# tesseract-robotics/trajopt

Measured on AMD Instinct MI355X. Metric: SQP iters/s (+ QP solves/s), 7-DOF x 30-wp x 1024-batch glass_upright, higher is better.
Workload: dtype f64; 1 GPU; config 1: glass_upright 7-DOF 30-waypoint, collision cost, batch=1024 random seeds per GPU; n_dof=7, n_steps=30, batch_per_gpu=1024, qp_n=572, qp_m=876, parallelism=seeds sharded, dp1

## Files before the change

### trajopt_amd/csrc/tmx_api.cpp

```cpp
#include <algorithm>
#include <cstddef>
#include <limits>
#include <string>
#include <vector>

#include "tmx_kernels.h"
#include "tmx_wave_kernels.h"
#include "tmx_wave_plan.h"
#include "tmx_row_perm.h"
#include "tmx_upload.h"

#ifdef TMX_HOST_EMU
#include <chrono>
thread_local tmx_emu_idx tmx_emu_threadIdx, tmx_emu_blockIdx, tmx_emu_blockDim, tmx_emu_gridDim;
thread_local double* tmx_emu_smem = nullptr;
double tmx_emu_now_ms()
{
  return std::chrono::duration<double, std::milli>(std::chrono::steady_clock::now().time_since_epoch()).count();
}
#else
#include <rccl/rccl.h>
#endif

#define HIPCHK(call)                                                                                                  \
// ... 1402 lines not shown
      const int c = L.wp_start[t + 1] - L.wp_start[t];
      for (int u = L.wp_start[t]; u < L.wp_start[t + 1]; ++u)
        pl.epos[L.wp_list[u]] = acc + (u - L.wp_start[t]);
      acc += c + (c & 1);
      rows_max = std::max(rows_max, c);
    }
    for (int r = 0; r < R; ++r)
      naux_max = std::max(naux_max, L.naux[r]);
    pl.setup_fast = (rows_max <= TMX_SETUP_COL && naux_max <= 2 && R <= 2 * TMX_QP_NT) ? 1 : 0;
    pl.polish_fast = 0;
    if (pl.setup_fast && dpart_fits(D, T) && R2 == 0)
    {
      DPart dp;
      dpart_make(T, dp);
      const size_t gn = (size_t)dp.Lmax * D, g_doubles = (size_t)dp.P * gn * dpart_gstride((int)gn);
      pl.polish_fast = polish_fast_doubles(T, D * T, R, NA, acc + TMX_SETUP_COL) <= g_doubles ? 1 : 0;
    }
    const size_t eval_room = tmx_eval_scratch_doubles(R, D * T, (int)L.vel_first.size(), L.n_costs, L.n_cnts);
    pl.step_fast = (pl.setup_fast && dpart_fits(D, T) && R >= 1 && 2 * (size_t)L.n_costs + 3 * (size_t)L.n_cnts + TMX_STEP_LOG_HEAD + 1 <= eval_room && R2 == 0 && D * T <= TMX_QP_NT && P.n_max + 1 <= TMX_STEP_CP_PASSES * TMX_QP_NT && P.flavor == 0 &&
                    !P.st && !P.band && !P.band_rows && !E.qp_dense && !P.use_time && P.n_fx == 0 && P.n_stencil == 0 && P.n_tt == 0 && P.n_tv == 0 &&
                    !(pl.coef_far & 2))
                       ? 1
                       : 0;
  }
  pl.smem_small = small_smem_bytes(L, P);
#if TMX_IS_DEVICE
  {
    std::vector<int> plan(TMX_WV_NT * TMX_WV_REC, 0);
    int gmax = 4, aux2 = 0, n3 = 0;
    if (hooks.wave == '1' && P.flavor == 0 && R2 == 0 && pl.coef_far == 0 && !E.qp_dense && !P.st && !P.band && !P.use_time && P.n_fx == 0 &&
        wave_plan_build(D, T, R, L.st.data(), L.naux.data(), plan.data(), &gmax, &aux2, &n3))
    {
      const size_t lds = std::max(pl.smem_small, wave_lds_doubles(D, T, R) * sizeof(double));
      if (lds <= 40 * 1024)
      {
        pl.plan.swap(plan);
        pl.wave_ok = 1;
        pl.wv_gmax = gmax;
        pl.wv_aux2 = aux2;
        pl.smem_wave = lds;
      }
    }
  }
#endif
  pl.smem_qp = qp_smem_bytes(D, T, R, NA, R2, pl.coef_far);
  if (P.tt_chain > 0 || P.tv_chain)
// ... 98 lines not shown
  UP(ls_link, L.ls_link);
  UP(ls_center, L.ls_center);
  UP(ls_radius, L.ls_radius);
  UP(ob_center, L.ob_center);
  UP(ob_radius, L.ob_radius);
  UP(ob_axis, L.ob_axis);
  UP(tv_owner, L.tv_owner);
  UP(tv_joint, L.tv_joint);
  UP(tv_first, L.tv_first);
  UP(tv_last, L.tv_last);
  UP(tv_coeff, L.tv_coeff);
  UP(tv_target, L.tv_target);
  UP(tv_up, L.tv_up);
  UP(tv_lo, L.tv_lo);
  UP(tt_owner, L.tt_owner);
  UP(tt_form, L.tt_form);
  UP(tt_slot, L.tt_slot);
  UP(tt_coeff, L.tt_coeff);
  UP(tt_limit, L.tt_limit);
  P.coef_far = pl.coef_far;
  P.setup_fast = pl.setup_fast;
  P.polish_fast = pl.polish_fast;
  P.step_fast = pl.step_fast;
  P.tt_place = pl.tt_place;
  P.wave_ok = pl.wave_ok;
  P.wv_gmax = pl.wv_gmax;
  P.wv_aux2 = pl.wv_aux2;
  if (!pl.row_perm.empty())
    UP(row_perm, pl.row_perm);
  UP(wp_pst, pl.pst);
  UP(row_epos, pl.epos);
  if (pl.wave_ok)
    UP(wv_plan, pl.plan);
#undef UP
  if (!ctx->dp)
  {
    void* p = nullptr;
    HIPCHK(hipMalloc(&p, sizeof(DevProblem)));
    ctx->dp = static_cast<DevProblem*>(p);
  }
  HIPCHK(hipMemcpy(ctx->dp, &P, sizeof(DevProblem), hipMemcpyHostToDevice));
  return TMX_OK;
}

static tmx_status configure_launch(tmx_ctx* ctx, const DevProblem& P, const Lowered& L, const EngineChoice& E, const Placement& pl, const UploadHooks& hooks)
{
// ... 1472 lines not shown
}

__attribute__((visibility("default"))) int tmx_debug_setup_fast(tmx_ctx* ctx)
{
  if (!ctx || !ctx->have_problem)
    return -1;
  return ctx->hp.setup_fast;
}

__attribute__((visibility("default"))) int tmx_debug_polish_fast(tmx_ctx* ctx)
{
  if (!ctx || !ctx->have_problem)
    return -1;
  return ctx->hp.polish_fast;
}

__attribute__((visibility("default"))) int tmx_debug_step_fast(tmx_ctx* ctx)
{
  if (!ctx || !ctx->have_problem)
    return -1;
  return ctx->hp.step_fast;
}

__attribute__((visibility("default"))) int tmx_debug_wave_ok(tmx_ctx* ctx)
{
  if (!ctx || !ctx->have_problem)
    return -1;
  return ctx->hp.wave_ok;
}

__attribute__((visibility("default"))) int tmx_debug_qp_dense(tmx_ctx* ctx)
{
  if (!ctx || !ctx->have_problem)
    return -1;
  return ctx->hp.qp_dense;
}

__attribute__((visibility("default"))) int tmx_debug_tt_chain(tmx_ctx* ctx)
{
  if (!ctx || !ctx->have_problem)
    return -1;
  return ctx->hp.tt_chain;
}

__attribute__((visibility("default"))) int tmx_debug_tv_chain(tmx_ctx* ctx)
{
// ... 23 lines not shown
```

### trajopt_amd/csrc/tmx_kernels.h

```cpp
#pragma once
#include "tmx_solve.h"
#include "tmx_step.h"
#include "tmx_generic.h"

#define TMX_WORK(smem, Bt) ((Bt)->ws_hbm ? (Bt)->ws_hbm + (size_t)blockIdx.x * (size_t)(Bt)->ws_hbm_stride : (smem))

template <bool HULL>
TMX_DEVFN void prepare_body(const DevProblem* P, const DevBatch* Bt)
{
  TMX_SMEM(smem);
  const int b = blockIdx.x, tid = threadIdx.x, NT = blockDim.x;
  const int NX = P->NX, D = P->D, R = P->R;
  const double* x0 = Bt->x0 + (size_t)b * NX;
  double* x = Bt->x + (size_t)b * NX;
  for (int v = tid; v < NX; v += NT)
  {
    const int j = v % D;
    double y = fmax(P->jl[j] + 1e-6, x0[v]);
    y = fmin(P->ju[j] - 1e-6, x0[v]);
    x[v] = (P->flavor == 1) ? x0[v] : y;
  }
  int* act = Bt->active + (size_t)b * R;
  for (int r = tid; r < R; r += NT)
    act[r] = 0;
// ... 348 lines not shown
TMX_DEVFN void sqp_step_block(const DevProblem* P, const DevBatch* Bt, int b, double* smem, int tid, int NT, double* chain_lds = nullptr)
{
  const int R = P->R, D = P->D, NX = P->NX;
  int* act = Bt->active + (size_t)b * R;
  double* coef = Bt->coef + (size_t)b * R * D;
  double* rhs = Bt->rhs + (size_t)b * R;
  double* x = Bt->x + (size_t)b * NX;
  double* xn = Bt->xnew + (size_t)b * NX;
  const double* xq = Bt->xq + (size_t)b * P->n_max;
#ifdef TMX_PROFILE
  long long tp0 = TMX_CLK();
  const long long wall0 = wall_clock64();
#endif
  if (P->sqp.max_time < 1e300)
  {
    if (tid == 0)
      sqp_time_limit_check(P, Bt, b);
    TMX_SYNC();
    if (Bt->phase[b] == PHASE_DONE)
      return;
  }
  if (Bt->phase[b] == PHASE_CONVEXIFY)
  {
    convexify_terms(P, x, act, coef, Bt->coef2 + (size_t)b * P->n_link * D, rhs, smem, tid, NT, Bt->rowc + (size_t)b * R, Bt->qdyn + (size_t)b * NX);
#ifdef TMX_PROFILE
    if (tid == 0)
    {
      const long long tnow = TMX_CLK();
      Bt->prof[(size_t)b * 16 + 4] += tnow - tp0;
      tp0 = tnow;
    }
#endif
#if TMX_IS_DEVICE
    if (TMX_UNI_B(!HBM && NT == TMX_QP_NT && P->step_fast != 0 && !(P->dbg_flags & 8) && TMX_FAST_ALLOWED))
    {
#if TMX_ADMM_OUTLINED && !(defined(TMX_PROFILE) && defined(TMX_FINE))
      unsigned lds_off = (unsigned)(size_t)smem;
      TMX_ASM_OPAQUE_SGPR(lds_off);
      qp_structure_fast_nl(P, Bt, b, lds_off);
#else
      qp_structure_fast(P, act, coef, Bt->dims + 4 * b, Bt->hashes + 4 * b, reinterpret_cast<int*>(smem), tid TMX_F5_ARGS(&tp0, Bt->prof + (size_t)b * 16));
#endif
    }
    else
#endif
    {
      QpWs cwd;
      qp_structure(P, act, coef, Bt->coef2 + (size_t)b * P->n_link * D, rhs, x, Bt->trust[b], Bt->merit + (size_t)b * P->n_cnts, Bt->dims + 4 * b,
                   Bt->hashes + 4 * b, nullptr, reinterpret_cast<int*>(smem), tid, NT, Bt->qdyn + (size_t)b * NX, compact_lists_of(cwd, P, Bt, b),
                   nullptr, nullptr, nullptr, nullptr TMX_F5_ARGS(&tp0, Bt->prof + (size_t)b * 16));
    }
#if TMX_LINK_ROWS
    if (P->flavor == 1)
      sqp2_begin_qp(P, Bt, b, smem, tid, NT);
#endif
  }
  TMX_SYNC();
#ifdef TMX_PROFILE
  if (tid == 0)
    Bt->prof[(size_t)b * 16 + 11] += TMX_CLK() - tp0;
#endif
  qp_solve_block<HBM, BANDK, false>(P, Bt, b, smem, tid, NT, chain_lds);
#ifdef TMX_PROFILE
  tp0 = TMX_CLK();
#endif
  for (int v = tid; v < NX; v += NT)
    xn[v] = xq[v];
  TMX_SYNC();
  evaluate_terms(P, xn, Bt->new_cost_vals + (size_t)b * P->n_costs, Bt->new_cnt_viols + (size_t)b * P->n_cnts, smem, tid, NT);
#if defined(TMX_PROFILE) && defined(TMX_FINE) && TMX_FINE == 5
  [[maybe_unused]] long long* const f5_tl = &tp0;
  [[maybe_unused]] long long* const f5_pc = Bt->prof + (size_t)b * 16;
#endif
  TMX_F5_TICK(13);
#if TMX_IS_DEVICE
  if (TMX_UNI_B(!HBM && NT == TMX_QP_NT && P->step_fast != 0 && !(P->dbg_flags & 8) && TMX_FAST_ALLOWED))
  {
#if TMX_ADMM_OUTLINED && !(defined(TMX_PROFILE) && defined(TMX_FINE))
    unsigned lds_off = (unsigned)(size_t)smem;
    TMX_ASM_OPAQUE_SGPR(lds_off);
    sqp_update_fast_nl(P, Bt, b, lds_off);
#else
    sqp_update_fast(P, Bt, b, smem, tid TMX_F5_ARGS(&tp0, Bt->prof + (size_t)b * 16));
#endif
  }
  else
#endif
#if TMX_LINK_ROWS
  if (P->flavor == 1)
    sqp2_update_block(P, Bt, b, smem, tid, NT);
  else
#endif
    sqp_update_block(P, Bt, b, smem, tid, NT TMX_F5_ARGS(&tp0, Bt->prof + (size_t)b * 16));
  TMX_SYNC();
#ifdef TMX_PROFILE
  if (tid == 0)
  {
    Bt->prof[(size_t)b * 16 + 12] += TMX_CLK() - tp0;
    Bt->prof[(size_t)b * 16 + 1] += wall_clock64() - wall0;
  }
#endif
}

TMX_KERNEL_LB2(TMX_QP_NT, TMX_QP_WGS_PER_CU) k_sqp_fused(const DevProblem* P, const DevBatch* Bt, int max_steps)
{
  TMX_SMEM(smem);
// ... 307 lines not shown
```

### trajopt_amd/csrc/tmx_step.h

```cpp
#pragma once
#include "tmx_solve.h"

#define TMX_STEP_CP_PASSES 6

#if TMX_IS_DEVICE
TMX_DEVFN void qp_structure_fast(const DevProblem* P, const int* active, const double* coef, int* dims, unsigned long long* hashes,
                                 int* iscratch, int tid TMX_F5_PARAMS)
{
  constexpr int NT = TMX_QP_NT;
  const int D = P->D, NX = P->NX, R = P->R;
  int* colptr = iscratch;
  int* rowref = colptr + P->n_max + 1;
  int* auxref = rowref + R;
  int* lact = auxref + R;
  int* lnaux = lact + R;
  int* ccount = lnaux + R;
  int acc_off = 2 * (P->n_max + 1) + 4 * R;
  acc_off += (acc_off & 1);
  unsigned long long* acc = reinterpret_cast<unsigned long long*>(iscratch + acc_off);
  int* scan = iscratch + acc_off + 16;
  int* nm = scan + TMX_STEP_CP_PASSES * (NT / 64);
  for (int r = tid; r < R; r += NT)
  {
    lact[r] = active[r] ? 1 : 0;
// ... 134 lines not shown
  };
  if (pv)
  {
    int pos = cp[0];
#pragma unroll
    for (int k = 0; k < TMX_SETUP_COL; ++k)
      if (mask & (1u << k))
      {
        row_term(rref[k], pos);
        ++pos;
      }
    row_term(mg + v, pos);
  }
  for (int r = tid; r < R; r += NT)
    if (lact[r])
      for (int k = 0; k < lnaux[r]; ++k)
      {
        const int col = auxref[r] + k;
        const int pos = colptr[col];
        row_term(rowref[r], pos);
        row_term(mg + col, pos + 1);
      }
  TMX_F5_TICK(6);
  unsigned long long hP = 0ULL, wsP = 0ULL;
  {
    const int pp_bytes = n + 1, pp_full = pp_bytes / 8, pp_rem = pp_bytes % 8;
    const int pi_full = P->nnzP / 8, pi_rem = P->nnzP % 8;
    auto p_term = [&](long long row, int run) {
      hP += tmx_hash_term(row, (uint64_t)run, 2);
      if (run < pi_full)
        wsP += tmx_hash_term(row, (uint64_t)run, 12);
      else if (run == pi_full && pi_rem > 0)
        wsP += tmx_hash_term((long long)((unsigned long long)row & ((1ULL << (8 * pi_rem)) - 1ULL)), (uint64_t)run, 12);
    };
    for (int c = tid; c <= n; c += NT)
    {
      int run = (c <= NX) ? P->p_colptr[c] : P->nnzP;
      const long long val = run;
      hP += tmx_hash_term(val, (uint64_t)c, 1);
      if (c < pp_full)
        wsP += tmx_hash_term(val, (uint64_t)c, 11);
      else if (c == pp_full && pp_rem > 0)
        wsP += tmx_hash_term((long long)((unsigned long long)val & ((1ULL << (8 * pp_rem)) - 1ULL)), (uint64_t)c, 11);
      if (c < NX)
      {
        if (c >= D && P->po[c - D] != 0.0)
        {
          p_term(c - D, run);
          ++run;
        }
        if (P->pd[c] != 0.0)
          p_term(c, run);
      }
    }
  }
  TMX_ATOMIC_ADD_U64(&acc[0], hP);
  TMX_ATOMIC_ADD_U64(&acc[1], hA);
  TMX_ATOMIC_ADD_U64(&acc[2], wsP);
  TMX_ATOMIC_ADD_U64(&acc[3], wsA);
  TMX_SYNC();
  if (tid == 0)
  {
    hashes[0] = acc[0];
    hashes[1] = acc[1];
    hashes[2] = acc[2];
    hashes[3] = acc[3];
  }
  TMX_SYNC();
}

TMX_DEVFN void sqp_update_fast(const DevProblem* P, const DevBatch* Bt, int b, double* smem, int tid TMX_F5_PARAMS)
{
  constexpr int NT = TMX_QP_NT;
  const int NX = P->NX, nc = P->n_costs, nv = P->n_cnts;
  double* model_cost = smem;
  double* model_viol = smem + nc;
  double* l_cost = model_viol + nv;
  double* l_new_cost = l_cost + nc;
  double* l_viol = l_new_cost + nc;
  double* l_new_viol = l_viol + nv;
  double* l_merit = l_new_viol + nv;
  double* head = l_merit + nv;
  double* cost_vals = Bt->cost_vals + (size_t)b * nc;
  double* cnt_viols = Bt->cnt_viols + (size_t)b * nv;
  const double* new_cost = Bt->new_cost_vals + (size_t)b * nc;
  const double* new_viol = Bt->new_cnt_viols + (size_t)b * nv;
  const double* merit = Bt->merit + (size_t)b * nv;
  const bool solved = Bt->cvx[b] == TMX_CVX_SOLVED && Bt->phase[b] != PHASE_DONE;
  if (solved)
    sqp_model_values<false>(P, Bt, b, Bt->xq + (size_t)b * P->n_max, smem, tid, NT);
  TMX_F5_TICK(14);
  for (int k = tid; k < nc; k += NT)
  {
    l_cost[k] = cost_vals[k];
    l_new_cost[k] = new_cost[k];
  }
  for (int k = tid; k < nv; k += NT)
  {
    l_viol[k] = cnt_viols[k];
    l_new_viol[k] = new_viol[k];
    l_merit[k] = merit[k];
  }
  if (tid == 0)
    head[TMX_STEP_LOG_HEAD] = 0.0;
  TMX_SYNC();
  if (tid == 0)
  {
    Bt->accept_flag[b] = 0;
    const DecideIo io = { l_cost, l_viol, l_new_cost, l_new_viol, l_merit, head };
    sqp_decide_io(P, Bt, b, model_cost, model_viol, io);
  }
  TMX_SYNC();
// ... 33 lines not shown
    for (int k = tid; k < nv; k += NT)
      cnt_viols[k] = l_new_viol[k];
  }
}

#if TMX_ADMM_OUTLINED
__device__ __attribute__((noinline)) static void qp_structure_fast_nl(const DevProblem* P_in, const DevBatch* Bt_in, int b_in, unsigned lds_in)
{
  const DevProblem* P = tmx_uniform_ptr(P_in);
  const DevBatch* Bt = tmx_uniform_ptr(Bt_in);
  const int b = __builtin_amdgcn_readfirstlane(b_in);
  const int tid = threadIdx.x;
  double* smem = (double*)(tmx_lds_d*)(size_t)(unsigned)__builtin_amdgcn_readfirstlane((int)lds_in);
  qp_structure_fast(P, Bt->active + (size_t)b * P->R, Bt->coef + (size_t)b * P->R * P->D, Bt->dims + 4 * b, Bt->hashes + 4 * b,
                    reinterpret_cast<int*>(smem), tid);
}
__device__ __attribute__((noinline)) static void sqp_update_fast_nl(const DevProblem* P_in, const DevBatch* Bt_in, int b_in, unsigned lds_in)
{
  const DevProblem* P = tmx_uniform_ptr(P_in);
  const DevBatch* Bt = tmx_uniform_ptr(Bt_in);
  const int b = __builtin_amdgcn_readfirstlane(b_in);
  const int tid = threadIdx.x;
  double* smem = (double*)(tmx_lds_d*)(size_t)(unsigned)__builtin_amdgcn_readfirstlane((int)lds_in);
  sqp_update_fast(P, Bt, b, smem, tid);
}
#endif
#endif
```

### trajopt_amd/csrc/tmx_terms.h

```cpp
#pragma once
#include "tmx_types.h"
#include "../../include/tmx_detmath.h"
#include "../../include/tmx_expr.h"
#include "../../include/tmx_geom.h"

#define TMX_EPS_FD 1e-5
#define TMX_CLEANUP_TOL 1e-7

struct Tf3
{
  double R[9];
  double t[3];
};

TMX_DEVFN void tf_from12(const double* a, Tf3& T)
{
  for (int r = 0; r < 3; ++r)
  {
    for (int c = 0; c < 3; ++c)
      T.R[3 * r + c] = a[4 * r + c];
    T.t[r] = a[4 * r + 3];
  }
}
TMX_DEVFN void tf_mul(const Tf3& A, const Tf3& B, Tf3& C)
{
  for (int r = 0; r < 3; ++r)
  {
    for (int c = 0; c < 3; ++c)
      C.R[3 * r + c] = A.R[3 * r + 0] * B.R[0 + c] + A.R[3 * r + 1] * B.R[3 + c] + A.R[3 * r + 2] * B.R[6 + c];
    C.t[r] = A.R[3 * r + 0] * B.t[0] + A.R[3 * r + 1] * B.t[1] + A.R[3 * r + 2] * B.t[2] + A.t[r];
  }
}
TMX_DEVFN void tf_inv(const Tf3& A, Tf3& C)
{
  for (int r = 0; r < 3; ++r)
    for (int c = 0; c < 3; ++c)
      C.R[3 * r + c] = A.R[3 * c + r];
  for (int r = 0; r < 3; ++r)
    C.t[r] = -(C.R[3 * r + 0] * A.t[0] + C.R[3 * r + 1] * A.t[1] + C.R[3 * r + 2] * A.t[2]);
}
TMX_DEVFN void tf_joint_motion(const double* ax, int type, double q, Tf3& T)
{
  for (int k = 0; k < 9; ++k)
    T.R[k] = 0.0;
  T.R[0] = T.R[4] = T.R[8] = 1.0;
  T.t[0] = T.t[1] = T.t[2] = 0.0;
  if (type == 0)
  {
    double c, s;
    tmx_sincos(q, &s, &c);
    const double v = 1.0 - c;
    const double x = ax[0], y = ax[1], z = ax[2];
    T.R[0] = c + x * x * v;
    T.R[1] = x * y * v - z * s;
    T.R[2] = x * z * v + y * s;
    T.R[3] = y * x * v + z * s;
    T.R[4] = c + y * y * v;
    T.R[5] = y * z * v - x * s;
    T.R[6] = z * x * v - y * s;
    T.R[7] = z * y * v + x * s;
    T.R[8] = c + z * z * v;
  }
  else
  {
    T.t[0] = ax[0] * q;
    T.t[1] = ax[1] * q;
    T.t[2] = ax[2] * q;
  }
}

template <class QAt, class Visit>
TMX_DEVFN void fk_link_visit(const DevProblem* P, QAt&& qat, int upto, Tf3& out, Visit&& visit)
{
  Tf3 T, O, M, U;
  tf_from12(P->base, T);
  for (int k = 0; k <= upto; ++k)
  {
    tf_from12(P->origin[k], O);
    tf_mul(T, O, U);
    visit(k, U);
    tf_joint_motion(P->axis[k], P->jtype[k], qat(k), M);
    tf_mul(U, M, T);
  }
  out = T;
}
template <class QAt>
TMX_DEVFN void fk_link_at(const DevProblem* P, QAt&& qat, int upto, Tf3& out)
{
  fk_link_visit(P, qat, upto, out, [](int, const Tf3&) {});
}
TMX_DEVFN void fk_link(const DevProblem* P, const double* q, int upto, Tf3& out)
// ... 161 lines not shown
__device__ __attribute__((noinline)) static int link_closest_b_nl(const double* c, const double* e, const double* oc, const double* oa, const double* ob,
                                                                  const double* mesh, double* p, double* q)
{
  return tmx_link_closest_to_obstacle_b(c, e, oc, oa, ob, mesh, p, q);
}
__device__ __attribute__((noinline)) static double swept_closest_b_nl(const double* ca, const double* e, const double* oc, const double* oa,
                                                                      const double* ob, const double* mesh, double* q, int* inside)
{
  return tmx_swept_closest_to_obstacle_b(ca, e, oc, oa, ob, mesh, q, inside);
}
__device__ __attribute__((noinline)) static int hull_closest_nl(const double* hv, int nv, const double* R0, const double* t0, const double* R1,
                                                                const double* t1, const double* oc, const double* oa, const double* ob,
                                                                const double* mesh, double* p, double* q, double* tau)
{
  return tmx_hull_closest_to_obstacle(hv, nv, R0, t0, R1, t1, oc, oa, ob, mesh, p, q, tau);
}
#else
#define link_closest_b_nl tmx_link_closest_to_obstacle_b
#define swept_closest_b_nl tmx_swept_closest_to_obstacle_b
#define hull_closest_nl tmx_hull_closest_to_obstacle
#endif

template <bool HULL = false>
TMX_DEVFN double contact_distance(const DevProblem* P, const double* q, int s, int o, double n[3], double pw[3])
{
  Tf3 L;
  const int link = P->ls_link[s];
  fk_link(P, q, link, L);
  if constexpr (HULL)
    if (P->n_ls_hull > 0 && P->ls_hull[2 * s + 1] > 0)
    {
      double pc[3], oq[3];
      const int inside = hull_closest_nl(P->hull + 3 * P->ls_hull[2 * s], P->ls_hull[2 * s + 1], L.R, L.t, nullptr, nullptr, P->ob_center + 3 * o,
                                         P->ob_axis + 3 * o, P->n_ob_box > 0 ? P->ob_box + 12 * o : nullptr, P->mesh, pc, oq, nullptr);
      const double len = tmx_contact_normal(pc, oq, inside, n);
      const double rs = P->ls_radius[s];
      for (int r = 0; r < 3; ++r)
        pw[r] = pc[r] + rs * n[r];
      return len - rs - P->ob_radius[o];
    }
  double c[3], d[3];
  for (int r = 0; r < 3; ++r)
    c[r] = L.R[3 * r + 0] * P->ls_center[3 * s + 0] + L.R[3 * r + 1] * P->ls_center[3 * s + 1] +
           L.R[3 * r + 2] * P->ls_center[3 * s + 2] + L.t[r];
  double oq[3];
  int inside = 0;
  if (P->n_ls_capsule > 0 || P->n_ob_box > 0)
  {
    double e[3], pc[3];
    bool capsule = false;
    if (P->n_ls_capsule > 0)
    {
      for (int r = 0; r < 3; ++r)
        e[r] = L.R[3 * r + 0] * P->ls_axis[3 * s + 0] + L.R[3 * r + 1] * P->ls_axis[3 * s + 1] + L.R[3 * r + 2] * P->ls_axis[3 * s + 2];
      capsule = P->ls_axis[3 * s + 0] != 0.0 || P->ls_axis[3 * s + 1] != 0.0 || P->ls_axis[3 * s + 2] != 0.0;
    }
    inside = link_closest_b_nl(c, capsule ? e : nullptr, P->ob_center + 3 * o, P->ob_axis + 3 * o,
                                            P->n_ob_box > 0 ? P->ob_box + 12 * o : nullptr, P->mesh, pc, oq);
    for (int r = 0; r < 3; ++r)
      c[r] = pc[r];
  }
  else
    tmx_obstacle_closest_to_point(P->ob_center + 3 * o, P->ob_axis + 3 * o, c, oq);
  (void)d;
  const double len = tmx_contact_normal(c, oq, inside, n);
  const double rs = P->ls_radius[s];
  for (int r = 0; r < 3; ++r)
    pw[r] = c[r] + rs * n[r];
  return len - rs - P->ob_radius[o];
}

struct LvsContact
{
  double distance, n[3], p_local[3], cc_time;
  double R0[9], R1[9];
};
TMX_DEVFN double lin_spaced_at(int size, double low, double high, int i)
{
  const int size1 = size - 1;
  const double step = (high - low) / (double)size1;
  const bool flip = fabs(high) < fabs(low);
  if (flip)
    return (i == 0) ? low : (high - (double)(size1 - i) * step);
  return (i == size1) ? high : (low + (double)i * step);
}
template <bool HULL = false>
TMX_DEVFN bool lvs_contact(const DevProblem* P, const double* q0, const double* q1, int r, LvsContact& c)
{
  const int s = P->slot_sub[r], o = P->slot_sub2[r], flags = P->slot_sub3[r];
  const int i = (flags >> 3) & 0x1FFF, kmax = flags >> 16;
  const bool fixed0 = flags & 1, fixed1 = flags & 2, cast = flags & 4;
  const double lvs = P->slot_aux3[r], margin = P->slot_aux1[r], buffer = P->slot_aux2[r];
// ... 1449 lines not shown
```

### trajopt_amd/csrc/tmx_types.h

```cpp
#pragma once
#include "../../include/tmx.h"
#include "tmx_platform.h"

enum
{
  SLOT_FIXED = 0,
  SLOT_CARTPOSE = 1,
  SLOT_JOINTPOS = 2,
  SLOT_COLLISION = 3,
  SLOT_JOINTPOS_INEQ = 4,
  SLOT_JOINTVEL = 5,
  SLOT_JOINTVEL_INEQ = 6,
  SLOT_COLLISION_LVS = 7,
  SLOT_FUNC = 9,
  SLOT_CARTVEL = 8,
  SLOT_JOINTVEL_TIME = 10,
  SLOT_TOTAL_TIME = 11
};
#ifndef TMX_LINK_ROWS
#define TMX_LINK_ROWS 1
#endif

enum
{
// ... 57 lines not shown
  int* ls_hull;
  double* hull;
  int n_ls_hull;
  int DK;
  int use_time;
  int n_tv;
  int *tv_owner, *tv_joint, *tv_first, *tv_last;
  double *tv_coeff, *tv_target, *tv_up, *tv_lo;
  int n_tt;
  int *tt_owner, *tt_form, *tt_slot;
  double *tt_coeff, *tt_limit;
  int wave_ok;
  int wv_gmax;
  int wv_aux2;
  int* wv_plan;
  int* row_perm;
  int dbg_flags;
  int tt_chain, tt_place;
  int tv_chain;
  int *wp_pst, *row_epos;
  int setup_fast;
  int polish_fast;
  int step_fast;
};
TMX_HOSTDEVFN int slot_is_diff(int kind) { return kind == SLOT_JOINTVEL || kind == SLOT_JOINTVEL_INEQ; }
#define TMX_TV_REC 5
TMX_HOSTDEVFN int fx_is_quad(int kind) { return kind == 0 || kind == 1 || kind == 3; }
TMX_HOSTDEVFN int fx_is_rows(int kind) { return kind == 2 || kind == 4; }

struct DevBatch
{
  int B, max_rec;
  double *x0, *x, *xnew;
  double *cost_vals, *cnt_viols, *new_cost_vals, *new_cnt_viols, *merit;
  double *trust, *total_cost, *prev_rho;
  int *phase, *iter, *merit_inc, *qp_fail, *status, *retval, *n_fe, *n_qp, *cvx, *prev_ok;
  int *active;
  double *coef, *rhs;
  double *qdyn;
  double *rowc;
  int *solver_init;
  double *coef2;
  int *dims;
  unsigned long long *hashes;
  int *prev_dims;
  unsigned long long *prev_ws;
// ... 42 lines not shown
```

### trajopt_amd/csrc/tmx_upload.h

```cpp
#pragma once
#include <cstddef>
#include <cstdlib>
#include <string>
#include <vector>

struct Lowered
{
  std::vector<int> kind, st, sub, sub2, owner, naux, iscnt, iseq;
  std::vector<double> objc, scale, aux1, aux2;
  std::vector<int> c2, sub3;
  std::vector<double> aux3;
  std::vector<int> aoff;
  std::vector<double> pd, po, pq, po2, po3;
  std::vector<int> p_colptr;
  std::vector<int> fx_t, fx_kind, fx_owner, fx_op0, fx_nops, fx_c0, fx_nout, fx_slot0, fx_ci, fx_ops;
  std::vector<double> fx_consts;
  std::vector<int> vel_first, vel_last, vel_cost, vel_kind, cp_t, cp_owner, cp_iscnt, cp_nrows, cp_idx, cp_slot0;
  std::vector<double> vel_coeffs, vel_targets, cp_coeff, cp_target;
  std::vector<int> tv_owner, tv_joint, tv_first, tv_last, tt_owner, tt_form, tt_slot;
  std::vector<double> tv_coeff, tv_target, tv_up, tv_lo, tt_coeff, tt_limit;
  std::vector<int> ls_link, ls_hull;
  std::vector<double> ls_center, ls_radius, ob_center, ob_radius, ob_axis, ls_axis, ob_box, hullv, mesh;
  std::vector<int> wp_start, wp_list;
  int R = 0, R2 = 0, NA = 0;
// ... 28 lines not shown
  static UploadHooks read()
  {
    auto first = [](const char* name) {
      const char* e = std::getenv(name);
      return e ? e[0] : '\0';
    };
    UploadHooks h;
    h.total_time_chain = first("TMX_TOTAL_TIME_CHAIN");
    h.vel_time_chain = first("TMX_VEL_TIME_CHAIN");
    h.force_coef_far = first("TMX_FORCE_COEF_FAR");
    h.force_compact = first("TMX_FORCE_COMPACT");
    h.row_perm = first("TMX_ROW_PERM");
    h.wave = first("TMX_WAVE");
    h.tt_place = first("TMX_TT_PLACE");
    const char* e = std::getenv("TMX_DENSE_QP_MAX_N");
    h.dense_qp_max_n = e ? std::max(1, std::atoi(e)) : 448;
    h.verbose = std::getenv("TMX_VERBOSE") != nullptr;
    return h;
  }
};

struct Placement
{
  int coef_far = 0, setup_fast = 0, polish_fast = 0, step_fast = 0, tt_place = 0;
  int wave_ok = 0, wv_gmax = 2, wv_aux2 = 0;
  std::vector<int> row_perm, pst, epos, plan;
  size_t smem_qp = 0, smem_small = 0, smem_wave = 0;
  size_t tt_scratch = 0;
};
```

Baseline: 170,200 SQP iters/s.

## Fuse term evaluation with model values in fast step path and tabulate P hash

Adds a merged fast path that evaluates cost and constraint terms together with the QP model values in one pass. It computes forward-kinematics frames once per waypoint in LDS with shared sin/cos and reuses them for collision and Cartesian terms. The P-matrix structure hash, which depends only on n, is now precomputed on the host per possible size and looked up instead of being recomputed each iteration. A convexify_fast routine that reuses cached frames for collision gradients is also added. Together these are meant to remove redundant FK and hashing work per SQP step, at the cost of extra LDS use and eligibility checks, with the old path kept as a fallback.

```diff
diff --git a/trajopt_amd/csrc/tmx_api.cpp b/trajopt_amd/csrc/tmx_api.cpp
--- a/trajopt_amd/csrc/tmx_api.cpp
+++ b/trajopt_amd/csrc/tmx_api.cpp
@@ -1448,6 +1448,22 @@
                     !(pl.coef_far & 2))
                        ? 1
                        : 0;
+    bool kinds_ok = true;
+    for (int k : L.kind)
+      kinds_ok = kinds_ok && tmx_step_eval_kind(k);
+    for (int k : L.vel_kind)
+      kinds_ok = kinds_ok && (k == 0 || k == 1);
+    const size_t qp_lds = qp_smem_bytes(D, T, R, NA, R2, pl.coef_far);
+    pl.eval_fast = (pl.step_fast && kinds_ok && qp_lds <= 160 * 1024 &&
+                    tmx_step_eval_doubles(R, D * T, (int)L.vel_first.size(), L.n_costs, L.n_cnts) * sizeof(double) <= qp_lds &&
+                    tmx_cvx_fast_doubles((int)L.cp_t.size(), D, D * T) * sizeof(double) <= qp_lds)
+                       ? 1
+                       : 0;
+    if (pl.eval_fast)
+    {
+      pl.p_hash.assign(2 * (size_t)(P.n_max - P.NX + 1), 0ULL);
+      tmx_build_p_hash_table(L.p_colptr.data(), L.pd.data(), L.po.data(), D, P.NX, P.n_max, P.nnzP, pl.p_hash.data());
+    }
   }
   pl.smem_small = small_smem_bytes(L, P);
 #if TMX_IS_DEVICE
@@ -1592,6 +1608,9 @@
   P.setup_fast = pl.setup_fast;
   P.polish_fast = pl.polish_fast;
   P.step_fast = pl.step_fast;
+  P.eval_fast = pl.eval_fast;
+  if (pl.eval_fast)
+    UP(p_hash, pl.p_hash);
   P.tt_place = pl.tt_place;
   P.wave_ok = pl.wave_ok;
   P.wv_gmax = pl.wv_gmax;
@@ -3110,6 +3129,13 @@
   return ctx->hp.step_fast;
 }
 
+__attribute__((visibility("default"))) int tmx_debug_eval_fast(tmx_ctx* ctx)
+{
+  if (!ctx || !ctx->have_problem)
+    return -1;
+  return ctx->hp.eval_fast;
+}
+
 __attribute__((visibility("default"))) int tmx_debug_wave_ok(tmx_ctx* ctx)
 {
   if (!ctx || !ctx->have_problem)
diff --git a/trajopt_amd/csrc/tmx_eval.h b/trajopt_amd/csrc/tmx_eval.h
--- /dev/null
+++ b/trajopt_amd/csrc/tmx_eval.h
@@ -0,0 +1,485 @@
+#pragma once
+#include "tmx_solve.h"
+
+TMX_HOSTDEVFN void p_hash_column(const int* p_colptr, const double* pd, const double* po, int D, int NX, int nnzP, int n, int c,
+                                 unsigned long long& hP, unsigned long long& wsP)
+{
+  const int pp_bytes = n + 1, pp_full = pp_bytes / 8, pp_rem = pp_bytes % 8;
+  const int pi_full = nnzP / 8, pi_rem = nnzP % 8;
+  auto p_term = [&](long long row, int run) {
+    hP += tmx_hash_term(row, (uint64_t)run, 2);
+    if (run < pi_full)
+      wsP += tmx_hash_term(row, (uint64_t)run, 12);
+    else if (run == pi_full && pi_rem > 0)
+      wsP += tmx_hash_term((long long)((unsigned long long)row & ((1ULL << (8 * pi_rem)) - 1ULL)), (uint64_t)run, 12);
+  };
+  int run = (c <= NX) ? p_colptr[c] : nnzP;
+  const long long val = run;
+  hP += tmx_hash_term(val, (uint64_t)c, 1);
+  if (c < pp_full)
+    wsP += tmx_hash_term(val, (uint64_t)c, 11);
+  else if (c == pp_full && pp_rem > 0)
+    wsP += tmx_hash_term((long long)((unsigned long long)val & ((1ULL << (8 * pp_rem)) - 1ULL)), (uint64_t)c, 11);
+  if (c < NX)
+  {
+    if (c >= D && po[c - D] != 0.0)
+    {
+      p_term(c - D, run);
+      ++run;
+    }
+    if (pd[c] != 0.0)
+      p_term(c, run);
+  }
+}
+
+static inline void tmx_build_p_hash_table(const int* p_colptr, const double* pd, const double* po, int D, int NX, int n_max, int nnzP,
+                                          unsigned long long* tab)
+{
+  for (int n = NX; n <= n_max; ++n)
+  {
+    unsigned long long hP = 0ULL, wsP = 0ULL;
+    for (int c = 0; c <= n; ++c)
+      p_hash_column(p_colptr, pd, po, D, NX, nnzP, n, c, hP, wsP);
+    tab[2 * (n - NX)] = hP;
+    tab[2 * (n - NX) + 1] = wsP;
+  }
+}
+
+TMX_HOSTDEVFN size_t tmx_step_eval_doubles(int R, int NX, int n_vel, int n_costs, int n_cnts)
+{
+  return (size_t)n_costs + (size_t)n_cnts + 2 * ((size_t)R + (size_t)(R + 1) / 2) + (size_t)n_vel * NX + (size_t)n_vel + 14 * (size_t)NX;
+}
+TMX_HOSTDEVFN bool tmx_step_eval_kind(int kind)
+{
+  return kind == SLOT_FIXED || kind == SLOT_CARTPOSE || kind == SLOT_JOINTPOS || kind == SLOT_JOINTPOS_INEQ || kind == SLOT_COLLISION;
+}
+
+#if TMX_IS_DEVICE
+#define TMX_EVAL_LDS_PTR(p) ((tmx_lds_d*)(size_t)(unsigned)__builtin_amdgcn_readfirstlane((int)(unsigned)(size_t)(p)))
+TMX_DEVFN void step_eval_fast(const DevProblem* P, const DevBatch* Bt, int b, double* smem, int tid)
+{
+  constexpr int NT = TMX_QP_NT;
+  const int D = P->D, NX = P->NX, R = P->R, T = P->T, nc = P->n_costs, nv = P->n_cnts, nvel = P->n_vel;
+  const double* xv = Bt->xnew + (size_t)b * NX;
+  const double* xq = Bt->xq + (size_t)b * P->n_max;
+  double* cost_out = Bt->new_cost_vals + (size_t)b * nc;
+  double* viol_out = Bt->new_cnt_viols + (size_t)b * nv;
+  const bool solved = TMX_UNI_B(Bt->cvx[b] == TMX_CVX_SOLVED && Bt->phase[b] != PHASE_DONE);
+  double* model_cost = smem;
+  double* model_viol = smem + nc;
+  double* xval = model_viol + nv;
+  int* xkeys = reinterpret_cast<int*>(xval + R);
+  double* mval = xval + R + (R + 1) / 2;
+  int* mkeys = reinterpret_cast<int*>(mval + R);
+  double* vterm = mval + R + (R + 1) / 2;
+  double* vsum = vterm + (size_t)nvel * NX;
+  tmx_lds_d* const SN = TMX_EVAL_LDS_PTR(vsum + nvel);
+  tmx_lds_d* const CS = SN + NX;
+  tmx_lds_d* const FR = CS + NX;
+  for (int v = tid; v < NX; v += NT)
+    if (P->jtype[v % D] == 0)
+    {
+      double s, c;
+      tmx_sincos(xv[v], &s, &c);
+      SN[v] = s;
+      CS[v] = c;
+    }
+  {
+    const int* act = Bt->active + (size_t)b * R;
+    const double* coef = Bt->coef + (size_t)b * R * D;
+    const double* rhs = Bt->rhs + (size_t)b * R;
+    QpWs wl;
+    qp_ws_carve(wl, smem, smem, Bt->qp_scratch + (size_t)b * Bt->qp_scratch_stride, D, T, R, P->NA, P->n_link, P->coef_far);
+    const int* aux_ref = wl.aux_ref;
+    for (int r = tid; r < R; r += NT)
+    {
+      const int kind = P->slot_kind[r];
+      const int t = P->slot_t[r];
+      if (kind == SLOT_JOINTPOS_INEQ)
+      {
+        const double pos = xv[t * D + P->slot_sub[r]] - P->slot_aux1[r];
+        const double e = (P->slot_sub2[r] == 0) ? (pos - P->slot_aux2[r]) * P->slot_scale[r] : ((pos * -1) + P->slot_aux2[r]) * P->slot_scale[r];
+        xval[r] = (e > 0) ? e : 0.0;
+      }
+      else if (kind == SLOT_JOINTPOS)
+      {
+        const double d = xv[t * D + P->slot_sub[r]] - P->slot_aux1[r];
+        xval[r] = fabs((d * d) * P->slot_scale[r]);
+      }
+      else if (kind == SLOT_FIXED)
+        xval[r] = 0.0;
+      xkeys[r] = (kind == SLOT_FIXED) ? -1 : (P->slot_iscnt[r] ? nc + P->slot_owner[r] : P->slot_owner[r]);
+      if (solved)
+      {
+        double vr = 0.0;
+        int key = -1;
+        if (kind != SLOT_FIXED && act[r])
+        {
+          if (P->slot_iscnt[r])
+          {
+            double aff = 0.0;
+            for (int j = 0; j < D; ++j)
+              aff += coef[r * D + j] * xq[t * D + j];
+            aff -= rhs[r];
+            vr = P->slot_eq[r] ? fabs(aff) : ((aff > 0) ? aff : 0.0);
+            key = nc + P->slot_owner[r];
+          }
+          else
+          {
+            double sacc = 0.0;
+            for (int k = 0; k < P->slot_naux[r]; ++k)
+              sacc += P->slot_objc[r] * xq[aux_ref[r] + k];
+            vr = sacc;
+            key = P->slot_owner[r];
+          }
+        }
+        mval[r] = vr;
+        mkeys[r] = key;
+      }
+    }
+  }
+  for (int v = 0; v < nvel; ++v)
+  {
+    const int pk = P->vel_kind[v];
+    const int first = P->vel_first[v], len = P->vel_last[v] - first + vel_len_adj<false>(pk);
+    for (int e = tid; e < D * len; e += NT)
+    {
+      const int j = e / len, i = first + e % len;
+      const double dv = pk ? xv[i * D + j] : (xv[(i + 1) * D + j] - xv[i * D + j]);
+      const double d = dv - P->vel_targets[v * TMX_MAX_DOF + j];
+      vterm[(size_t)v * NX + e] = (d * d) * P->vel_coeffs[v * TMX_MAX_DOF + j];
+    }
+  }
+  TMX_SYNC();
+  for (int t = tid; t < T; t += NT)
+  {
+    Tf3 F, O, M, U;
+    tf_from12(P->base, F);
+    for (int k = 0; k < D; ++k)
+    {
+      tf_from12(P->origin[k], O);
+      tf_mul(F, O, U);
+      const int type = P->jtype[k];
+      double s = 0.0, c = 1.0;
+      if (type == 0)
+      {
+        s = SN[t * D + k];
+        c = CS[t * D + k];
+      }
+      tf_joint_motion_sc(P->axis[k], type, xv[t * D + k], s, c, M);
+      tf_mul(U, M, F);
+      tmx_lds_d* const o = FR + (size_t)(t * D + k) * 12;
+#pragma unroll
+      for (int i = 0; i < 9; ++i)
+        o[i] = F.R[i];
+#pragma unroll
+      for (int i = 0; i < 3; ++i)
+        o[9 + i] = F.t[i];
+    }
+  }
+  for (int v = (tid + NT - 64) % NT; v < nvel; v += NT)
+  {
+    const int cnt = D * (P->vel_last[v] - P->vel_first[v] + vel_len_adj<false>(P->vel_kind[v]));
+    double sacc = 0;
+    for (int e = 0; e < cnt; ++e)
+      sacc += vterm[(size_t)v * NX + e];
+    vsum[v] = sacc;
+  }
+  TMX_SYNC();
+  auto frame_at = [&](int t, int k, Tf3& L) {
+    tmx_lds_d* const o = FR + (size_t)(t * D + k) * 12;
+#pragma unroll
+    for (int i = 0; i < 9; ++i)
+      L.R[i] = o[i];
+#pragma unroll
+    for (int i = 0; i < 3; ++i)
+      L.t[i] = o[9 + i];
+  };
+  for (int r = tid; r < R; r += NT)
+    if (P->slot_kind[r] == SLOT_COLLISION)
+    {
+      const int s = P->slot_sub[r];
+      Tf3 L;
+      frame_at(P->slot_t[r], P->ls_link[s], L);
+      double n[3], pw[3];
+      const double dist = contact_distance_at<false>(P, L, s, P->slot_sub2[r], n, pw);
+      const double margin = P->slot_aux1[r];
+      double v = 0.0;
+      if (!(dist > margin + P->slot_aux2[r]))
+      {
+        const double pv = margin - dist;
+        v = ((pv > 0) ? pv : 0.0) * P->slot_objc[r];
+      }
+      xval[r] = v;
+    }
+  for (int c = tid; c < P->n_cp; c += NT)
+  {
+    Tf3 tgt, tinv, L, Tl, src;
+    tf_from12(P->cp_target + 12 * c, tgt);
+    tf_inv(tgt, tinv);
+    frame_at(P->cp_t[c], D - 1, L);
+    tf_from12(P->tool, Tl);
+    tf_mul(L, Tl, src);
+    double err[6], ax[3], ang;
+    transform_error(tinv, src, err, ax, ang);
+    const int s0 = P->cp_slot0[c];
+    for (int i = 0; i < P->cp_nrows[c]; ++i)
+    {
+      const int ix = P->cp_idx[6 * c + i];
+      const double e = (ix == 0) ? err[0] : (ix == 1) ? err[1] : (ix == 2) ? err[2] : (ix == 3) ? err[3] : (ix == 4) ? err[4] : err[5];
+      const double cc = P->cp_coeff[6 * c + i];
+      xval[s0 + i] = P->cp_iscnt[c] ? fabs(e * cc) : fabs(e) * cc;
+    }
+  }
+  TMX_SYNC();
+  for (int k = tid; k < nc + nv; k += NT)
+  {
+    double acc = 0.0;
+    for (int r = P->own_lo[k]; r <= P->own_hi[k]; ++r)
+      if (xkeys[r] == k)
+        acc += xval[r];
+    if (k < nc)
+    {
+      for (int v = 0; v < nvel; ++v)
+        if (P->vel_cost[v] == k)
+          acc += vsum[v];
+      cost_out[k] = acc;
+    }
+    else
+      viol_out[k - nc] = acc;
+  }
+  if (solved)
+    for (int k = (tid + NT - 64) % NT; k < nc + nv; k += NT)
+    {
+      double acc = 0.0;
+      for (int r = P->own_lo[k]; r <= P->own_hi[k]; ++r)
+        if (mkeys[r] == k)
+          acc += mval[r];
+      if (k < nc)
+      {
+        for (int v = 0; v < nvel; ++v)
+          if (P->vel_cost[v] == k)
+            acc += vsum[v];
+        model_cost[k] = acc;
+      }
+      else
+        model_viol[k - nc] = acc;
+    }
+  TMX_SYNC();
+}
+#endif
+
+TMX_HOSTDEVFN size_t tmx_cvx_fast_doubles(int n_cp, int D, int NX) { return tmx_cvx_scratch_doubles(n_cp, D) + 28 * (size_t)NX; }
+
+#if TMX_IS_DEVICE
+TMX_DEVFN void convexify_fast(const DevProblem* P, const double* xv, int* active, double* coef, double* rhs, double* scratch, int tid)
+{
+  constexpr int NT = TMX_QP_NT;
+  const int D = P->D, NX = P->NX, T = P->T, n_cp = P->n_cp;
+  double* rec = scratch;
+  double* errv = rec + (size_t)n_cp * (D + 1) * 7;
+  double* Jm = errv + (size_t)n_cp * 6;
+  tmx_lds_d* const SN = TMX_EVAL_LDS_PTR(scratch + tmx_cvx_scratch_doubles(n_cp, D));
+  tmx_lds_d* const CS = SN + NX;
+  tmx_lds_d* const SNP = CS + NX;
+  tmx_lds_d* const CSP = SNP + NX;
+  tmx_lds_d* const FU = CSP + NX;
+  tmx_lds_d* const FL = FU + (size_t)NX * 12;
+  auto frame_put = [&](tmx_lds_d* o, const Tf3& F) {
+#pragma unroll
+    for (int i = 0; i < 9; ++i)
+      o[i] = F.R[i];
+#pragma unroll
+    for (int i = 0; i < 3; ++i)
+      o[9 + i] = F.t[i];
+  };
+  auto frame_get = [&](tmx_lds_d* o, Tf3& F) {
+#pragma unroll
+    for (int i = 0; i < 9; ++i)
+      F.R[i] = o[i];
+#pragma unroll
+    for (int i = 0; i < 3; ++i)
+      F.t[i] = o[9 + i];
+  };
+  for (int v = tid; v < NX; v += NT)
+    if (P->jtype[v % D] == 0)
+    {
+      double s, c;
+      tmx_sincos(xv[v], &s, &c);
+      SN[v] = s;
+      CS[v] = c;
+      if (n_cp > 0)
+      {
+        tmx_sincos(xv[v] + TMX_EPS_FD, &s, &c);
+        SNP[v] = s;
+        CSP[v] = c;
+      }
+    }
+  TMX_SYNC();
+  for (int t = tid; t < T; t += NT)
+  {
+    Tf3 F, O, M, U;
+    tf_from12(P->base, F);
+    for (int k = 0; k < D; ++k)
+    {
+      tf_from12(P->origin[k], O);
+      tf_mul(F, O, U);
+      frame_put(FU + (size_t)(t * D + k) * 12, U);
+      const int type = P->jtype[k];
+      double s = 0.0, c = 1.0;
+      if (type == 0)
+      {
+        s = SN[t * D + k];
+        c = CS[t * D + k];
+      }
+      tf_joint_motion_sc(P->axis[k], type, xv[t * D + k], s, c, M);
+      tf_mul(U, M, F);
+      frame_put(FL + (size_t)(t * D + k) * 12, F);
+    }
+  }
+  for (int item = (tid + NT - 64) % NT; item < n_cp * (D + 1); item += NT)
+  {
+    const int c = item / (D + 1), k = item % (D + 1);
+    const int t = P->cp_t[c];
+    const double* q = xv + t * D;
+    Tf3 tgt, tinv, src, pp;
+    tf_from12(P->cp_target + 12 * c, tgt);
+    tf_inv(tgt, tinv);
+    {
+      Tf3 F, O, M, U, Tl;
+      tf_from12(P->base, F);
+      for (int j = 0; j < D; ++j)
+      {
+        tf_from12(P->origin[j], O);
+        tf_mul(F, O, U);
+        const int type = P->jtype[j];
+        double s = 0.0, cs = 1.0;
+        if (type == 0)
+        {
+          s = (j == k) ? SNP[t * D + j] : SN[t * D + j];
+          cs = (j == k) ? CSP[t * D + j] : CS[t * D + j];
+        }
+        tf_joint_motion_sc(P->axis[j], type, (j == k) ? q[j] + TMX_EPS_FD : q[j], s, cs, M);
+        tf_mul(U, M, F);
+      }
+      tf_from12(P->tool, Tl);
+      tf_mul(F, Tl, src);
+    }
+    tf_mul(tinv, src, pp);
+    double ax[3], ang;
+    if (k < D)
+      rot_err_decomposed(pp.R, ax, ang);
+    else
+    {
+      double err[6];
+      transform_error(tinv, src, err, ax, ang);
+      for (int r = 0; r < 6; ++r)
+        errv[c * 6 + r] = err[r];
+    }
+    double* o = rec + (size_t)item * 7;
+    for (int r = 0; r < 3; ++r)
+    {
+      o[r] = pp.t[r];
+      o[3 + r] = ax[r];
+    }
+    o[6] = ang;
+  }
+  TMX_SYNC();
+  for (int item = tid; item < n_cp * D; item += NT)
+  {
+    const int c = item / D, k = item % D;
+    const double* o0 = rec + ((size_t)c * (D + 1) + D) * 7;
+    const double* o1 = rec + ((size_t)c * (D + 1) + k) * 7;
+    const double a0 = o0[6], a1 = o1[6];
+    double a1c = a1;
+    if (a1 > M_PI_2 && a0 < -M_PI_2)
+      a1c = a1 - 2.0 * M_PI;
+    else if (a1 < -M_PI_2 && a0 > M_PI_2)
+      a1c = a1 + 2.0 * M_PI;
+    for (int i = 0; i < P->cp_nrows[c]; ++i)
+    {
+      const int r = P->cp_idx[6 * c + i];
+      const double diff = (r < 3) ? o1[r] - o0[r] : o1[r] * a1c - o0[r] * a0;
+      Jm[((size_t)c * 6 + i) * D + k] = diff / TMX_EPS_FD;
+    }
+  }
+  for (int r = tid; r < P->R; r += NT)
+  {
+    if (P->slot_kind[r] != SLOT_COLLISION)
+      continue;
+    const int t = P->slot_t[r];
+    const double* q = xv + t * D;
+    const int s = P->slot_sub[r], o = P->slot_sub2[r];
+    const int link = P->ls_link[s];
+    double n[3], pw[3];
+    Tf3 L;
+    frame_get(FL + (size_t)(t * D + link) * 12, L);
+    const double dist = contact_distance_at<false>(P, L, s, o, n, pw);
+    const double margin = P->slot_aux1[r];
+    if (dist > margin + P->slot_aux2[r])
+    {
+      active[r] = 0;
+      for (int k = 0; k < D; ++k)
+        coef[r * D + k] = 0.0;
+      rhs[r] = 0.0;
+      continue;
+    }
+    double* grad = coef + (size_t)r * D;
+    double gq = 0.0;
+    for (int k = 0; k <= link; ++k)
+    {
+      Tf3 F;
+      frame_get(FU + (size_t)(t * D + k) * 12, F);
+      const double g = contact_grad_col(P, k, F, pw, n);
+      grad[k] = g;
+      gq += g * q[k];
+    }
+    for (int k = link + 1; k < D; ++k)
+    {
+      const double g = -1.0 * (n[0] * 0.0 + n[1] * 0.0 + n[2] * 0.0);
+      grad[k] = g;
+      gq += g * q[k];
+    }
+    const double c_dist = (0.0 + (-gq)) + dist;
+    const double viol_const = margin - c_dist;
+    if (P->slot_iscnt[r])
+    {
+      const double cc = P->slot_scale[r];
+      for (int k = 0; k < D; ++k)
+        coef[r * D + k] = (-grad[k]) * cc;
+      rhs[r] = -(viol_const * cc);
+    }
+    else
+    {
+      for (int k = 0; k < D; ++k)
+        coef[r * D + k] = -grad[k];
+      rhs[r] = -viol_const;
+    }
+    active[r] = 1;
+  }
+  TMX_SYNC();
+  for (int item = tid; item < n_cp * 6; item += NT)
+  {
+    const int c = item / 6, i = item % 6;
+    if (i >= P->cp_nrows[c])
+      continue;
+    const double* q = xv + P->cp_t[c] * D;
+    const double* Jr = Jm + ((size_t)c * 6 + i) * D;
+    const double y = errv[c * 6 + P->cp_idx[6 * c + i]];
+    double dot = 0.0;
+    for (int k = 0; k < D; ++k)
+      dot += Jr[k] * q[k];
+    const double cc = P->cp_coeff[6 * c + i];
+    const int r = P->cp_slot0[c] + i;
+    const double constant = (y - dot) * cc;
+    for (int k = 0; k < D; ++k)
+    {
+      const double jv = Jr[k];
+      coef[r * D + k] = (fabs(jv) > TMX_CLEANUP_TOL) ? jv * cc : 0.0;
+    }
+    rhs[r] = -constant;
+    active[r] = 1;
+  }
+  TMX_SYNC();
+}
+#endif
diff --git a/trajopt_amd/csrc/tmx_kernels.h b/trajopt_amd/csrc/tmx_kernels.h
--- a/trajopt_amd/csrc/tmx_kernels.h
+++ b/trajopt_amd/csrc/tmx_kernels.h
@@ -394,7 +394,20 @@
   }
   if (Bt->phase[b] == PHASE_CONVEXIFY)
   {
-    convexify_terms(P, x, act, coef, Bt->coef2 + (size_t)b * P->n_link * D, rhs, smem, tid, NT, Bt->rowc + (size_t)b * R, Bt->qdyn + (size_t)b * NX);
+#if TMX_IS_DEVICE
+    if (TMX_UNI_B(!HBM && NT == TMX_QP_NT && P->step_fast != 0 && P->eval_fast != 0 && !(P->dbg_flags & (8 | 16)) && TMX_FAST_ALLOWED))
+    {
+#if TMX_ADMM_OUTLINED && !(defined(TMX_PROFILE) && defined(TMX_FINE))
+      unsigned lds_off = (unsigned)(size_t)smem;
+      TMX_ASM_OPAQUE_SGPR(lds_off);
+      convexify_fast_nl(P, Bt, b, lds_off);
+#else
+      convexify_fast(P, x, act, coef, rhs, smem, tid);
+#endif
+    }
+    else
+#endif
+      convexify_terms(P, x, act, coef, Bt->coef2 + (size_t)b * P->n_link * D, rhs, smem, tid, NT, Bt->rowc + (size_t)b * R, Bt->qdyn + (size_t)b * NX);
 #ifdef TMX_PROFILE
     if (tid == 0)
     {
@@ -439,21 +452,33 @@
   for (int v = tid; v < NX; v += NT)
     xn[v] = xq[v];
   TMX_SYNC();
-  evaluate_terms(P, xn, Bt->new_cost_vals + (size_t)b * P->n_costs, Bt->new_cnt_viols + (size_t)b * P->n_cnts, smem, tid, NT);
 #if defined(TMX_PROFILE) && defined(TMX_FINE) && TMX_FINE == 5
   [[maybe_unused]] long long* const f5_tl = &tp0;
   [[maybe_unused]] long long* const f5_pc = Bt->prof + (size_t)b * 16;
 #endif
-  TMX_F5_TICK(13);
-#if TMX_IS_DEVICE
-  if (TMX_UNI_B(!HBM && NT == TMX_QP_NT && P->step_fast != 0 && !(P->dbg_flags & 8) && TMX_FAST_ALLOWED))
+#if TMX_IS_DEVICE
+  const bool step_fast = TMX_UNI_B(!HBM && NT == TMX_QP_NT && P->step_fast != 0 && !(P->dbg_flags & 8) && TMX_FAST_ALLOWED);
+  const bool merged = step_fast && TMX_UNI_B(P->eval_fast != 0 && !(P->dbg_flags & 16));
+  if (!merged)
+#endif
+  {
+    evaluate_terms(P, xn, Bt->new_cost_vals + (size_t)b * P->n_costs, Bt->new_cnt_viols + (size_t)b * P->n_cnts, smem, tid, NT);
+    TMX_F5_TICK(13);
+  }
+#if TMX_IS_DEVICE
+  if (step_fast)
   {
 #if TMX_ADMM_OUTLINED && !(defined(TMX_PROFILE) && defined(TMX_FINE))
     unsigned lds_off = (unsigned)(size_t)smem;
     TMX_ASM_OPAQUE_SGPR(lds_off);
     sqp_update_fast_nl(P, Bt, b, lds_off);
 #else
-    sqp_update_fast(P, Bt, b, smem, tid TMX_F5_ARGS(&tp0, Bt->prof + (size_t)b * 16));
+    if (merged)
+    {
+      step_eval_fast(P, Bt, b, smem, tid);
+      TMX_F5_TICK(13);
+    }
+    sqp_update_fast(P, Bt, b, smem, tid, merged TMX_F5_ARGS(&tp0, Bt->prof + (size_t)b * 16));
 #endif
   }
   else
diff --git a/trajopt_amd/csrc/tmx_step.h b/trajopt_amd/csrc/tmx_step.h
--- a/trajopt_amd/csrc/tmx_step.h
+++ b/trajopt_amd/csrc/tmx_step.h
@@ -1,5 +1,6 @@
 #pragma once
 #include "tmx_solve.h"
+#include "tmx_eval.h"
 
 #define TMX_STEP_CP_PASSES 6
 
@@ -180,54 +181,30 @@
         row_term(mg + col, pos + 1);
       }
   TMX_F5_TICK(6);
-  unsigned long long hP = 0ULL, wsP = 0ULL;
-  {
-    const int pp_bytes = n + 1, pp_full = pp_bytes / 8, pp_rem = pp_bytes % 8;
-    const int pi_full = P->nnzP / 8, pi_rem = P->nnzP % 8;
-    auto p_term = [&](long long row, int run) {
-      hP += tmx_hash_term(row, (uint64_t)run, 2);
-      if (run < pi_full)
-        wsP += tmx_hash_term(row, (uint64_t)run, 12);
-      else if (run == pi_full && pi_rem > 0)
-        wsP += tmx_hash_term((long long)((unsigned long long)row & ((1ULL << (8 * pi_rem)) - 1ULL)), (uint64_t)run, 12);
-    };
+  const bool p_tab = TMX_UNI_B(P->eval_fast != 0 && !(P->dbg_flags & 16));
+  if (!p_tab)
+  {
+    unsigned long long hP = 0ULL, wsP = 0ULL;
     for (int c = tid; c <= n; c += NT)
-    {
-      int run = (c <= NX) ? P->p_colptr[c] : P->nnzP;
-      const long long val = run;
-      hP += tmx_hash_term(val, (uint64_t)c, 1);
-      if (c < pp_full)
-        wsP += tmx_hash_term(val, (uint64_t)c, 11);
-      else if (c == pp_full && pp_rem > 0)
-        wsP += tmx_hash_term((long long)((unsigned long long)val & ((1ULL << (8 * pp_rem)) - 1ULL)), (uint64_t)c, 11);
-      if (c < NX)
-      {
-        if (c >= D && P->po[c - D] != 0.0)
-        {
-          p_term(c - D, run);
-          ++run;
-        }
-        if (P->pd[c] != 0.0)
-          p_term(c, run);
-      }
-    }
-  }
-  TMX_ATOMIC_ADD_U64(&acc[0], hP);
+      p_hash_column(P->p_colptr, P->pd, P->po, D, NX, P->nnzP, n, c, hP, wsP);
+    TMX_ATOMIC_ADD_U64(&acc[0], hP);
+    TMX_ATOMIC_ADD_U64(&acc[2], wsP);
+  }
   TMX_ATOMIC_ADD_U64(&acc[1], hA);
-  TMX_ATOMIC_ADD_U64(&acc[2], wsP);
   TMX_ATOMIC_ADD_U64(&acc[3], wsA);
   TMX_SYNC();
   if (tid == 0)
   {
-    hashes[0] = acc[0];
+    const unsigned long long* e = P->p_hash + 2 * (size_t)(n - NX);
+    hashes[0] = p_tab ? e[0] : acc[0];
     hashes[1] = acc[1];
-    hashes[2] = acc[2];
+    hashes[2] = p_tab ? e[1] : acc[2];
     hashes[3] = acc[3];
   }
   TMX_SYNC();
 }
 
-TMX_DEVFN void sqp_update_fast(const DevProblem* P, const DevBatch* Bt, int b, double* smem, int tid TMX_F5_PARAMS)
+TMX_DEVFN void sqp_update_fast(const DevProblem* P, const DevBatch* Bt, int b, double* smem, int tid, bool have_model TMX_F5_PARAMS)
 {
   constexpr int NT = TMX_QP_NT;
   const int NX = P->NX, nc = P->n_costs, nv = P->n_cnts;
@@ -245,7 +222,7 @@
   const double* new_viol = Bt->new_cnt_viols + (size_t)b * nv;
   const double* merit = Bt->merit + (size_t)b * nv;
   const bool solved = Bt->cvx[b] == TMX_CVX_SOLVED && Bt->phase[b] != PHASE_DONE;
-  if (solved)
+  if (solved && !have_model)
     sqp_model_values<false>(P, Bt, b, Bt->xq + (size_t)b * P->n_max, smem, tid, NT);
   TMX_F5_TICK(14);
   for (int k = tid; k < nc; k += NT)
@@ -325,7 +302,19 @@
   const int b = __builtin_amdgcn_readfirstlane(b_in);
   const int tid = threadIdx.x;
   double* smem = (double*)(tmx_lds_d*)(size_t)(unsigned)__builtin_amdgcn_readfirstlane((int)lds_in);
-  sqp_update_fast(P, Bt, b, smem, tid);
+  const bool merged = TMX_UNI_B(P->eval_fast != 0 && !(P->dbg_flags & 16));
+  if (merged)
+    step_eval_fast(P, Bt, b, smem, tid);
+  sqp_update_fast(P, Bt, b, smem, tid, merged);
+}
+__device__ __attribute__((noinline)) static void convexify_fast_nl(const DevProblem* P_in, const DevBatch* Bt_in, int b_in, unsigned lds_in)
+{
+  const DevProblem* P = tmx_uniform_ptr(P_in);
+  const DevBatch* Bt = tmx_uniform_ptr(Bt_in);
+  const int b = __builtin_amdgcn_readfirstlane(b_in);
+  const int tid = threadIdx.x;
+  double* smem = (double*)(tmx_lds_d*)(size_t)(unsigned)__builtin_amdgcn_readfirstlane((int)lds_in);
+  convexify_fast(P, Bt->x + (size_t)b * P->NX, Bt->active + (size_t)b * P->R, Bt->coef + (size_t)b * P->R * P->D, Bt->rhs + (size_t)b * P->R, smem, tid);
 }
 #endif
 #endif
diff --git a/trajopt_amd/csrc/tmx_terms.h b/trajopt_amd/csrc/tmx_terms.h
--- a/trajopt_amd/csrc/tmx_terms.h
+++ b/trajopt_amd/csrc/tmx_terms.h
@@ -39,7 +39,7 @@
   for (int r = 0; r < 3; ++r)
     C.t[r] = -(C.R[3 * r + 0] * A.t[0] + C.R[3 * r + 1] * A.t[1] + C.R[3 * r + 2] * A.t[2]);
 }
-TMX_DEVFN void tf_joint_motion(const double* ax, int type, double q, Tf3& T)
+TMX_DEVFN void tf_joint_motion_sc(const double* ax, int type, double q, double s, double c, Tf3& T)
 {
   for (int k = 0; k < 9; ++k)
     T.R[k] = 0.0;
@@ -47,8 +47,6 @@
   T.t[0] = T.t[1] = T.t[2] = 0.0;
   if (type == 0)
   {
-    double c, s;
-    tmx_sincos(q, &s, &c);
     const double v = 1.0 - c;
     const double x = ax[0], y = ax[1], z = ax[2];
     T.R[0] = c + x * x * v;
@@ -67,6 +65,13 @@
     T.t[1] = ax[1] * q;
     T.t[2] = ax[2] * q;
   }
+}
+TMX_DEVFN void tf_joint_motion(const double* ax, int type, double q, Tf3& T)
+{
+  double c = 1.0, s = 0.0;
+  if (type == 0)
+    tmx_sincos(q, &s, &c);
+  tf_joint_motion_sc(ax, type, q, s, c, T);
 }
 
 template <class QAt, class Visit>
@@ -274,11 +279,8 @@
 #endif
 
 template <bool HULL = false>
-TMX_DEVFN double contact_distance(const DevProblem* P, const double* q, int s, int o, double n[3], double pw[3])
-{
-  Tf3 L;
-  const int link = P->ls_link[s];
-  fk_link(P, q, link, L);
+TMX_DEVFN double contact_distance_at(const DevProblem* P, const Tf3& L, int s, int o, double n[3], double pw[3])
+{
   if constexpr (HULL)
     if (P->n_ls_hull > 0 && P->ls_hull[2 * s + 1] > 0)
     {
@@ -320,6 +322,14 @@
   for (int r = 0; r < 3; ++r)
     pw[r] = c[r] + rs * n[r];
   return len - rs - P->ob_radius[o];
+}
+template <bool HULL = false>
+TMX_DEVFN double contact_distance(const DevProblem* P, const double* q, int s, int o, double n[3], double pw[3])
+{
+  Tf3 L;
+  const int link = P->ls_link[s];
+  fk_link(P, q, link, L);
+  return contact_distance_at<HULL>(P, L, s, o, n, pw);
 }
 
 struct LvsContact
diff --git a/trajopt_amd/csrc/tmx_types.h b/trajopt_amd/csrc/tmx_types.h
--- a/trajopt_amd/csrc/tmx_types.h
+++ b/trajopt_amd/csrc/tmx_types.h
@@ -103,6 +103,8 @@
   int setup_fast;
   int polish_fast;
   int step_fast;
+  unsigned long long* p_hash;
+  int eval_fast;
 };
 TMX_HOSTDEVFN int slot_is_diff(int kind) { return kind == SLOT_JOINTVEL || kind == SLOT_JOINTVEL_INEQ; }
 #define TMX_TV_REC 5
diff --git a/trajopt_amd/csrc/tmx_upload.h b/trajopt_amd/csrc/tmx_upload.h
--- a/trajopt_amd/csrc/tmx_upload.h
+++ b/trajopt_amd/csrc/tmx_upload.h
@@ -74,9 +74,10 @@
 
 struct Placement
 {
-  int coef_far = 0, setup_fast = 0, polish_fast = 0, step_fast = 0, tt_place = 0;
+  int coef_far = 0, setup_fast = 0, polish_fast = 0, step_fast = 0, eval_fast = 0, tt_place = 0;
   int wave_ok = 0, wv_gmax = 2, wv_aux2 = 0;
   std::vector<int> row_perm, pst, epos, plan;
+  std::vector<unsigned long long> p_hash;
   size_t smem_qp = 0, smem_small = 0, smem_wave = 0;
   size_t tt_scratch = 0;
 };
```

Result: faster. 174,300 SQP iters/s, median of 6 (+2.4%).
